# nka77/DAHiTra

Measured on AMD Instinct MI355X. Metric: image-pairs/s (256x256) train step, 1/2/4/8 MI355X + CPU ref, higher is better.
Workload: dtype bf16; 1 GPU; LEVIR-CD 256x256 synthetic pairs, base_transformer_pos_s4, bf16, batch 32 per GPU (global 32), fwd+focal+bwd+allreduce+AdamW; net_G=base_transformer_pos_s4, global_batch=32, img_size=256, parallelism=dp1, hip_graph=True, step_form=one graph (AdamW inside), attn_dtype=bf16

## Files before the change

dahitra_amd/csrc/norm.hip:

```cpp
#include "common.h"

namespace {

constexpr int BN_MAXG = 4;
__global__ void bn_finalize_kernel(const float* __restrict__ partial, int ntiles, int CP, int C, int G,
                                   double count, const float* __restrict__ gamma,
                                   const float* __restrict__ beta, float* __restrict__ running_mean,
                                   float* __restrict__ running_var, float momentum, float eps,
                                   float* __restrict__ mean_out, float* __restrict__ invstd_out,
                                   float* __restrict__ scale_out, float* __restrict__ shift_out,
                                   long long* __restrict__ nbt) {
    __shared__ double sm[BN_MAXG], sv[BN_MAXG], ps[4], pq[4];
    const int c = blockIdx.x;
    if (nbt && c == 0 && threadIdx.x == 0) *nbt += G;
    const int lane = threadIdx.x & 63, w = threadIdx.x >> 6, wpg = 4 / G;
    const int g = w / wpg, slice = w % wpg;
    const int tpg = ntiles / G;
    {
        double s = 0.0, q = 0.0, s2 = 0.0, q2 = 0.0;
        const float* p0 = partial + ((size_t)0 * CP + c) * ntiles + (size_t)g * tpg;
        const float* p1 = partial + ((size_t)1 * CP + c) * ntiles + (size_t)g * tpg;
        const int step = 64 * wpg;
        int t = slice * 64 + lane;
#pragma unroll 4
        for (; t + step < tpg; t += 2 * step) {
            s += (double)p0[t]; q += (double)p1[t];
            s2 += (double)p0[t + step]; q2 += (double)p1[t + step];
        }
        if (t < tpg) { s += (double)p0[t]; q += (double)p1[t]; }
        s += s2; q += q2;
#pragma unroll
        for (int o = 32; o > 0; o >>= 1) {
            s += __shfl_xor(s, o, 64);
            q += __shfl_xor(q, o, 64);
        }
        if (lane == 0) { ps[w] = s; pq[w] = q; }
        __syncthreads();
        if (lane == 0 && slice == 0) {
            s = 0.0; q = 0.0;
            for (int k = 0; k < wpg; ++k) { s += ps[g * wpg + k]; q += pq[g * wpg + k]; }
            const double mean = s / count;
            double var = q / count - mean * mean;
            if (var < 0.0) var = 0.0;
            const float invstd = (float)(1.0 / sqrt(var + (double)eps));
            const float sc = gamma[c] * invstd;
            mean_out[g * C + c] = (float)mean;
            invstd_out[g * C + c] = invstd;
            scale_out[g * C + c] = sc;
            shift_out[g * C + c] = beta[c] - (float)mean * sc;
            sm[g] = mean;
            sv[g] = count > 1.0 ? var * count / (count - 1.0) : var;
        }
    }
// ... 943 lines not shown
                              float momentum, float eps, float* mean, float* invstd, float* scale, float* shift,
                              long long* num_batches_tracked, void* stream) {
    DH_REQUIRE_BN_GROUPS("bn_finalize", groups);
    DH_REQUIRE(ntiles % groups == 0, "bn_finalize: ntiles=%d not divisible by groups=%d", ntiles, groups);
    hipLaunchKernelGGL(bn_finalize_kernel, dim3(C), dim3(256), 0, ST(stream), partial, ntiles, CP, C, groups, count,
                       gamma, beta, running_mean, running_var, momentum, eps, mean, invstd, scale, shift,
                       num_batches_tracked);
    DH_CHECK_LAUNCH("bn_finalize");
    return 0;
}

extern "C" int dh_bn_eval_params(const float* gamma, const float* beta, const float* running_mean,
                                 const float* running_var, float eps, int C, float* scale, float* shift,
                                 void* stream) {
    hipLaunchKernelGGL(bn_eval_params_kernel, dim3(dh_cdiv(C, 64)), dim3(64), 0, ST(stream), gamma, beta,
                       running_mean, running_var, eps, C, scale, shift);
    DH_CHECK_LAUNCH("bn_eval_params");
    return 0;
}

static int bn_apply_impl(int dtype, const void* x, const void* residual, void* y, const float* scale, const float* shift, long npix,
                         int C, int groups, int act, unsigned char* relu_bits, void* stream, const float* res_scale = nullptr,
                         const float* res_shift = nullptr) {
    const int V = dtype == DH_DTYPE_BF16 ? 8 : 4;
    DH_REQUIRE_BN_GROUPS("bn_apply", groups);
    DH_REQUIRE(C % V == 0 && npix % groups == 0, "bn_apply: C=%d npix=%ld groups=%d", C, npix, groups);
    DH_REQUIRE(!relu_bits || act == DH_ACT_RELU, "bn_apply: the ReLU mask bytes go with act = DH_ACT_RELU");
    DH_REQUIRE(!res_scale == !res_shift && (!res_scale || residual), "bn_apply: res_scale and res_shift go together, with a residual");
    const long nvec = npix * C / V, gvec = nvec / groups;
    (void)gvec;
    if (dtype == DH_DTYPE_BF16)
        launch_bn_apply<bf16>(x, residual, y, scale, shift, nvec, C, groups, act, ST(stream), relu_bits, res_scale, res_shift);
    else launch_bn_apply<float>(x, residual, y, scale, shift, nvec, C, groups, act, ST(stream), relu_bits, res_scale, res_shift);
    DH_CHECK_LAUNCH("bn_apply");
    return 0;
}
extern "C" int dh_bn_apply(int dtype, const void* x, const void* residual, void* y, const float* scale,
                           const float* shift, long npix, int C, int groups, int act, void* stream) {
    return bn_apply_impl(dtype, x, residual, y, scale, shift, npix, C, groups, act, nullptr, stream);
}
extern "C" int dh_bn_apply_bits(int dtype, const void* x, const void* residual, void* y, const float* scale, const float* shift,
                                long npix, int C, int groups, int act, unsigned char* relu_bits, void* stream) {
    DH_REQUIRE(relu_bits, "bn_apply_bits: relu_bits missing");
    return bn_apply_impl(dtype, x, residual, y, scale, shift, npix, C, groups, act, relu_bits, stream);
}

extern "C" int dh_bn_apply_res_affine(int dtype, const void* x, const void* residual, const float* res_scale, const float* res_shift,
                                      void* y, const float* scale, const float* shift, long npix, int C, int groups, int act,
                                      unsigned char* relu_bits, void* stream) {
    DH_REQUIRE(residual && res_scale && res_shift, "bn_apply_res_affine: residual, res_scale and res_shift are all required");
    return bn_apply_impl(dtype, x, residual, y, scale, shift, npix, C, groups, act, relu_bits, stream, res_scale, res_shift);
}

extern "C" long dh_stem_pool_bn_bwd_workspace_size(int C, int groups) { return (long)(768 / groups) * groups * 2 * C * 4; }
extern "C" int dh_stem_pool_bn_bwd_plus(const unsigned char* argmax, const void* dpool, const void* extra, const void* y,
                                        const float* mask_scale, const float* mask_shift, const float* mean, const float* invstd,
                                        const float* gamma, int N, int H, int W, int C, int groups, void* d, float* coef,
                                        float* dgamma, float* dbeta, int accumulate, void* workspace, void* stream);
extern "C" int dh_stem_pool_bn_bwd(const unsigned char* argmax, const void* dpool, const void* y, const float* mask_scale,
                                   const float* mask_shift, const float* mean, const float* invstd, const float* gamma, int N,
                                   int H, int W, int C, int groups, void* d, float* coef, float* dgamma, float* dbeta,
                                   int accumulate, void* workspace, void* stream) {
    return dh_stem_pool_bn_bwd_plus(argmax, dpool, nullptr, y, mask_scale, mask_shift, mean, invstd, gamma, N, H, W, C, groups, d,
                                    coef, dgamma, dbeta, accumulate, workspace, stream);
}
extern "C" int dh_stem_pool_bn_bwd_plus(const unsigned char* argmax, const void* dpool, const void* extra, const void* y,
                                        const float* mask_scale, const float* mask_shift, const float* mean, const float* invstd,
                                        const float* gamma, int N, int H, int W, int C, int groups, void* d, float* coef,
                                        float* dgamma, float* dbeta, int accumulate, void* workspace, void* stream) {
    DH_REQUIRE(C % 8 == 0 && 256 % (C / 8) == 0 && 2 * C <= 256, "stem_pool_bn_bwd: unsupported C=%d", C);
    DH_REQUIRE(groups >= 1 && groups <= BN_MAXG && N % groups == 0, "stem_pool_bn_bwd: N=%d groups=%d", N, groups);
    const int bpg = 768 / groups, OH = (H + 2 - 3) / 2 + 1, OW = (W + 2 - 3) / 2 + 1;
    float* partial = reinterpret_cast<float*>(workspace);
    hipLaunchKernelGGL(pool_bn_bwd_reduce_kernel, dim3(groups * bpg), dim3(256), 0, ST(stream), argmax, (const bf16*)dpool,
                       (const bf16*)extra, (const bf16*)y, mask_scale, mask_shift, (bf16*)d, partial, N / groups, H, W, C, OH, OW, bpg);
    hipLaunchKernelGGL(bn_bwd_finalize_coef_kernel, dim3(C), dim3(64 * groups), 0, ST(stream), partial, bpg, groups, C, mean, invstd,
                       gamma, 1.0f / (float)((long)(N / groups) * H * W), coef, dgamma, dbeta, accumulate);
    DH_CHECK_LAUNCH("stem_pool_bn_bwd");
    return 0;
}

extern "C" long dh_bn_bwd_workspace_size(long npix, int C, int groups) {
    const int bpg = 1024 / groups;
    return ((long)groups * bpg * 2 * C + (long)groups * 2 * C) * 4;
}

static int bn_bwd_impl(int dtype, const void* dout, const void* out_relu, bool bits, const void* x, const float* mean,
                       const float* invstd, const float* gamma, long npix, int C, int groups, void* dx,
                       void* dres, float* dgamma, float* dbeta, int accumulate, const float* mask_scale,
                       const float* mask_shift, void* workspace, void* stream) {
    DH_REQUIRE_BN_GROUPS("bn_bwd", groups);
    DH_REQUIRE(!(out_relu && mask_scale), "bn_bwd: give the ReLU mask either as out_relu or as mask_scale/shift");
    DH_REQUIRE(!bits || out_relu, "bn_bwd: mask bytes missing");
    const int V = dtype == DH_DTYPE_BF16 ? 8 : 4;
    DH_REQUIRE(C % V == 0 && (256 * V) % C == 0, "bn_bwd: unsupported C=%d", C);
    DH_REQUIRE(npix % groups == 0, "bn_bwd: npix=%ld not divisible by groups=%d", npix, groups);
    const int bpg = 1024 / groups;
    const long ppg = npix / groups;
    float* partial = reinterpret_cast<float*>(workspace);
    float* sums = partial + (long)groups * bpg * 2 * C;
    const long nvec = npix * C / V;
    if (dtype == DH_DTYPE_BF16) {
        launch_bn_bwd_reduce<bf16>(dout, out_relu, x, mean, invstd, C, ppg, bpg, groups, partial, mask_scale, mask_shift, ST(stream), bits);
        hipLaunchKernelGGL(bn_bwd_finalize_kernel, dim3(C), dim3(64 * groups), 0, ST(stream), partial, bpg, groups, C, sums,
                           dgamma, dbeta, accumulate);
        launch_bn_bwd_apply<bf16>(dout, out_relu, x, mean, invstd, gamma, sums, ppg, nvec, C, groups, dx, dres, mask_scale,
                                  mask_shift, ST(stream), bits);
    } else {
        launch_bn_bwd_reduce<float>(dout, out_relu, x, mean, invstd, C, ppg, bpg, groups, partial, mask_scale, mask_shift, ST(stream), bits);
        hipLaunchKernelGGL(bn_bwd_finalize_kernel, dim3(C), dim3(64 * groups), 0, ST(stream), partial, bpg, groups, C, sums,
                           dgamma, dbeta, accumulate);
        launch_bn_bwd_apply<float>(dout, out_relu, x, mean, invstd, gamma, sums, ppg, nvec, C, groups, dx, dres, mask_scale,
                                   mask_shift, ST(stream), bits);
    }
    DH_CHECK_LAUNCH("bn_bwd");
    return 0;
}
extern "C" int dh_bn_bwd(int dtype, const void* dout, const void* out_relu, const void* x, const float* mean,
                         const float* invstd, const float* gamma, long npix, int C, int groups, void* dx,
                         void* dres, float* dgamma, float* dbeta, int accumulate, const float* mask_scale,
                         const float* mask_shift, void* workspace, void* stream) {
    return bn_bwd_impl(dtype, dout, out_relu, false, x, mean, invstd, gamma, npix, C, groups, dx, dres, dgamma, dbeta, accumulate,
                       mask_scale, mask_shift, workspace, stream);
}
extern "C" int dh_bn_bwd_bits(int dtype, const void* dout, const unsigned char* relu_bits, const void* x, const float* mean,
                              const float* invstd, const float* gamma, long npix, int C, int groups, void* dx,
                              void* dres, float* dgamma, float* dbeta, int accumulate, void* workspace, void* stream) {
    DH_REQUIRE(relu_bits, "bn_bwd_bits: relu_bits missing");
// ... 171 lines not shown
```

dahitra_amd/csrc/pointwise.hip:

```cpp
#include "common.h"

namespace {

inline int ew_grid(long n, int block) {
    long g = (n + block - 1) / block;
    return (int)(g > 8192 ? 8192 : (g < 1 ? 1 : g));
}
#define GSL(i, n) for (long i = (long)blockIdx.x * blockDim.x + threadIdx.x; i < (n); i += (long)gridDim.x * blockDim.x)

template <typename T>
__global__ void nchw_to_nhwc_kernel(const float* __restrict__ src, T* __restrict__ dst, int N, int C, long HW, int CP) {
    const long total = (long)N * HW * CP;
    GSL(i, total) {
        const int c = (int)(i % CP);
        const long p = (i / CP) % HW;
        const long n = i / (CP * HW);
        stf(dst + i, c < C ? src[(n * C + c) * HW + p] : 0.f);
    }
}
template <typename T>
__global__ void nchw_to_nhwc_piece_kernel(const float* __restrict__ src, T* __restrict__ dst, int N, int C, long HW) {
    constexpr int V = V16<T>::N;
    const long total = (long)N * HW;
    GSL(i, total) {
        const long p = i % HW, n = i / HW;
        float v[V];
#pragma unroll
        for (int c = 0; c < V; ++c) v[c] = c < C ? src[(n * C + c) * HW + p] : 0.f;
        stv(dst + i * V, v);
    }
}
template <typename T>
__global__ void nhwc_to_nchw_kernel(const T* __restrict__ src, float* __restrict__ dst, int N, int C, long HW) {
    const long total = (long)N * HW * C;
    GSL(i, total) {
        const long p = i % HW;
        const int c = (int)((i / HW) % C);
        const long n = i / (HW * C);
        dst[i] = ldf(src + (n * HW + p) * C + c);
    }
}

template <typename T, int CP>
__global__ __launch_bounds__(256) void head_dgrad3x3_kernel(const T* __restrict__ dy, const float* __restrict__ w_oihw,
                                                            T* __restrict__ dx, int N, int H, int W, int NC) {
    __shared__ __attribute__((aligned(16))) float sw[9 * 8 * 32];
    for (int i = threadIdx.x; i < 9 * NC * 32; i += blockDim.x) {
        const int ci = i & 31, co = (i >> 5) % NC, tap = i / (32 * NC);
        sw[i] = w_oihw[((size_t)co * 32 + ci) * 9 + tap];
    }
    __syncthreads();
    const long total = (long)N * H * W;
    for (long px = (long)blockIdx.x * blockDim.x + threadIdx.x; px < total; px += (long)gridDim.x * blockDim.x) {
// ... 1097 lines not shown
    DH_REQUIRE(C % V == 0, "cat_halves: C=%d must be a multiple of %d", C, V);
    const long n = P * (2 * C / V);
    if (dtype == DH_DTYPE_BF16) {
        if (inverse) hipLaunchKernelGGL((cat_halves_kernel<bf16, true>), dim3(ew_grid(n, 256)), dim3(256), 0, ST(stream), (bf16*)t, (bf16*)cat, C, P);
        else hipLaunchKernelGGL((cat_halves_kernel<bf16, false>), dim3(ew_grid(n, 256)), dim3(256), 0, ST(stream), (bf16*)t, (bf16*)cat, C, P);
    } else {
        if (inverse) hipLaunchKernelGGL((cat_halves_kernel<float, true>), dim3(ew_grid(n, 256)), dim3(256), 0, ST(stream), (float*)t, (float*)cat, C, P);
        else hipLaunchKernelGGL((cat_halves_kernel<float, false>), dim3(ew_grid(n, 256)), dim3(256), 0, ST(stream), (float*)t, (float*)cat, C, P);
    }
    DH_CHECK_LAUNCH("cat_halves");
    return 0;
}
extern "C" int dh_add(int dtype, const void* a, const void* b, void* y, long n, void* stream) {
    DH_REQUIRE(n % 4 == 0, "add: n must be a multiple of 4");
    const long nv = n / 4;
    if (dtype == DH_DTYPE_BF16 && n % 8 == 0) hipLaunchKernelGGL(add16_kernel<bf16>, dim3(ew_grid(n / 8, 256)), dim3(256), 0, ST(stream), (const bf16*)a, (const bf16*)b, (bf16*)y, n / 8);
    else if (dtype == DH_DTYPE_BF16) hipLaunchKernelGGL(add_kernel<bf16>, dim3(ew_grid(nv, 256)), dim3(256), 0, ST(stream), (const bf16*)a, (const bf16*)b, (bf16*)y, nv);
    else hipLaunchKernelGGL(add_kernel<float>, dim3(ew_grid(nv, 256)), dim3(256), 0, ST(stream), (const float*)a, (const float*)b, (float*)y, nv);
    DH_CHECK_LAUNCH("add");
    return 0;
}
extern "C" int dh_add_pos(int dtype, const void* x, const float* pos, void* y, int N, long HW, int C, void* stream) {
    const long n = (long)N * HW * C;
    if (dtype == DH_DTYPE_BF16 && C % 8 == 0) hipLaunchKernelGGL(add_pos16_kernel<bf16>, dim3(ew_grid(n / 8, 256)), dim3(256), 0, ST(stream), (const bf16*)x, pos, (bf16*)y, N, HW, C);
    else if (dtype == DH_DTYPE_BF16) hipLaunchKernelGGL(add_pos_kernel<bf16>, dim3(ew_grid(n, 256)), dim3(256), 0, ST(stream), (const bf16*)x, pos, (bf16*)y, N, HW, C);
    else hipLaunchKernelGGL(add_pos_kernel<float>, dim3(ew_grid(n, 256)), dim3(256), 0, ST(stream), (const float*)x, pos, (float*)y, N, HW, C);
    DH_CHECK_LAUNCH("add_pos");
    return 0;
}
extern "C" int dh_add_pos_bwd(int dtype, const void* dy, float* dpos, int N, long HW, int C, int accumulate, void* stream) {
    const long n = HW * C;
    if (dtype == DH_DTYPE_BF16 && C == 32) hipLaunchKernelGGL(add_pos_bwd32_kernel, dim3((unsigned)((HW + 15) / 16)), dim3(256), 0, ST(stream), (const bf16*)dy, dpos, N, HW, accumulate);
    else if (dtype == DH_DTYPE_BF16) hipLaunchKernelGGL(add_pos_bwd_kernel<bf16>, dim3(ew_grid(n, 256)), dim3(256), 0, ST(stream), (const bf16*)dy, dpos, N, HW, C, accumulate);
    else hipLaunchKernelGGL(add_pos_bwd_kernel<float>, dim3(ew_grid(n, 256)), dim3(256), 0, ST(stream), (const float*)dy, dpos, N, HW, C, accumulate);
    DH_CHECK_LAUNCH("add_pos_bwd");
    return 0;
}
extern "C" int dh_act_bwd(int dtype, const void* dy, const void* ref, void* dx, long n, int act, void* stream) {
    DH_REQUIRE(n % 4 == 0 && (act == DH_ACT_RELU || act == DH_ACT_GELU), "act_bwd: bad arguments");
    const long nv = n / 4;
    if (dtype == DH_DTYPE_BF16 && n % 8 == 0) hipLaunchKernelGGL(act_bwd16_kernel<bf16>, dim3(ew_grid(n / 8, 256)), dim3(256), 0, ST(stream), (const bf16*)dy, (const bf16*)ref, (bf16*)dx, n / 8, act);
    else if (dtype == DH_DTYPE_BF16) hipLaunchKernelGGL(act_bwd_kernel<bf16>, dim3(ew_grid(nv, 256)), dim3(256), 0, ST(stream), (const bf16*)dy, (const bf16*)ref, (bf16*)dx, nv, act);
    else hipLaunchKernelGGL(act_bwd_kernel<float>, dim3(ew_grid(nv, 256)), dim3(256), 0, ST(stream), (const float*)dy, (const float*)ref, (float*)dx, nv, act);
    DH_CHECK_LAUNCH("act_bwd");
    return 0;
}
extern "C" int dh_maxpool3x3s2_fwd(int dtype, const void* x, void* y, unsigned char* argmax, int N, int H, int W, int C,
                                   const float* bn_scale, const float* bn_shift, int groups, void* stream) {
    DH_REQUIRE(!bn_scale || (bn_shift && groups > 0 && N % groups == 0), "maxpool: bn_scale needs bn_shift and groups | N");
    const int V = dtype == DH_DTYPE_BF16 ? 8 : 4;
    DH_REQUIRE(C % V == 0, "maxpool: C=%d must be a multiple of %d", C, V);
    const int OH = (H + 2 - 3) / 2 + 1, OW = (W + 2 - 3) / 2 + 1;
    const long n = (long)N * OH * OW * (C / V);
    if (dtype == DH_DTYPE_BF16) hipLaunchKernelGGL(maxpool_fwd_kernel<bf16>, dim3(ew_grid(n, 256)), dim3(256), 0, ST(stream), (const bf16*)x, (bf16*)y, argmax, N, H, W, C, OH, OW, bn_scale, bn_shift, groups);
    else hipLaunchKernelGGL(maxpool_fwd_kernel<float>, dim3(ew_grid(n, 256)), dim3(256), 0, ST(stream), (const float*)x, (float*)y, argmax, N, H, W, C, OH, OW, bn_scale, bn_shift, groups);
    DH_CHECK_LAUNCH("maxpool_fwd");
    return 0;
}
extern "C" int dh_maxpool3x3s2_bwd(int dtype, const unsigned char* argmax, const void* dy, void* dx, int N, int H, int W, int C, void* stream) {
    const int V = dtype == DH_DTYPE_BF16 ? 8 : 4;
    DH_REQUIRE(C % V == 0, "maxpool: C=%d must be a multiple of %d", C, V);
    const int OH = (H + 2 - 3) / 2 + 1, OW = (W + 2 - 3) / 2 + 1;
    const long n = (long)N * ((H + 1) / 2) * ((W + 1) / 2) * (C / V);
    if (dtype == DH_DTYPE_BF16) hipLaunchKernelGGL(maxpool_bwd_kernel<bf16>, dim3(ew_grid(n, 256)), dim3(256), 0, ST(stream), argmax, (const bf16*)dy, (bf16*)dx, N, H, W, C, OH, OW);
    else hipLaunchKernelGGL(maxpool_bwd_kernel<float>, dim3(ew_grid(n, 256)), dim3(256), 0, ST(stream), argmax, (const float*)dy, (float*)dx, N, H, W, C, OH, OW);
    DH_CHECK_LAUNCH("maxpool_bwd");
    return 0;
}
extern "C" int dh_upsample2_nearest_fwd(int dtype, const void* x, void* y, int N, int H, int W, int C, void* stream) {
    const int V = dtype == DH_DTYPE_BF16 ? 8 : 4;
    DH_REQUIRE(C % V == 0, "upsample2: C=%d must be a multiple of %d", C, V);
    const long n = (long)N * 4 * H * W * (C / V);
    if (dtype == DH_DTYPE_BF16) hipLaunchKernelGGL(up2_fwd_kernel<bf16>, dim3(ew_grid(n, 256)), dim3(256), 0, ST(stream), (const bf16*)x, (bf16*)y, N, H, W, C);
    else hipLaunchKernelGGL(up2_fwd_kernel<float>, dim3(ew_grid(n, 256)), dim3(256), 0, ST(stream), (const float*)x, (float*)y, N, H, W, C);
    DH_CHECK_LAUNCH("up2_fwd");
    return 0;
}
extern "C" int dh_upsample2_nearest_bwd(int dtype, const void* dy, void* dx, int N, int H, int W, int C, void* stream) {
    const int V = dtype == DH_DTYPE_BF16 ? 8 : 4;
    DH_REQUIRE(C % V == 0, "upsample2: C=%d must be a multiple of %d", C, V);
    const long n = (long)N * H * W * (C / V);
    if (dtype == DH_DTYPE_BF16) hipLaunchKernelGGL(up2_bwd_kernel<bf16>, dim3(ew_grid(n, 256)), dim3(256), 0, ST(stream), (const bf16*)dy, (bf16*)dx, N, H, W, C);
    else hipLaunchKernelGGL(up2_bwd_kernel<float>, dim3(ew_grid(n, 256)), dim3(256), 0, ST(stream), (const float*)dy, (float*)dx, N, H, W, C);
    DH_CHECK_LAUNCH("up2_bwd");
    return 0;
}
extern "C" int dh_absdiff_upsample4_fwd(int dtype, const void* a, const void* b, void* y, int N, int H, int W, int C, void* stream) {
    const int V = dtype == DH_DTYPE_BF16 ? 8 : 4;
    DH_REQUIRE(C % V == 0, "absdiff_upsample4: C=%d must be a multiple of %d", C, V);
    const long n = (long)N * H * W * (C / V);
    if (dtype == DH_DTYPE_BF16) hipLaunchKernelGGL(absdiff_up4_fwd_kernel<bf16>, dim3(ew_grid(n, 256)), dim3(256), 0, ST(stream), (const bf16*)a, (const bf16*)b, (bf16*)y, N, H, W, C);
    else hipLaunchKernelGGL(absdiff_up4_fwd_kernel<float>, dim3(ew_grid(n, 256)), dim3(256), 0, ST(stream), (const float*)a, (const float*)b, (float*)y, N, H, W, C);
    DH_CHECK_LAUNCH("absdiff_up4_fwd");
    return 0;
}
extern "C" int dh_absdiff_upsample4_bwd(int dtype, const void* a, const void* b, const void* dy, void* da, void* db, int N, int H, int W, int C, void* stream) {
    const int V = dtype == DH_DTYPE_BF16 ? 8 : 4;
    DH_REQUIRE(C % V == 0, "absdiff_upsample4: C=%d must be a multiple of %d", C, V);
    const long n = (long)N * H * W * (C / V);
    if (dtype == DH_DTYPE_BF16) hipLaunchKernelGGL(absdiff_up4_bwd_kernel<bf16>, dim3(ew_grid(n, 256)), dim3(256), 0, ST(stream), (const bf16*)a, (const bf16*)b, (const bf16*)dy, (bf16*)da, (bf16*)db, N, H, W, C);
    else hipLaunchKernelGGL(absdiff_up4_bwd_kernel<float>, dim3(ew_grid(n, 256)), dim3(256), 0, ST(stream), (const float*)a, (const float*)b, (const float*)dy, (float*)da, (float*)db, N, H, W, C);
    DH_CHECK_LAUNCH("absdiff_up4_bwd");
    return 0;
}
extern "C" int dh_absdiff_up4_combine(const float* partial, const void* a, const void* b, void* da, void* db, int N, int H, int W,
                                      void* stream) {
    DH_REQUIRE(H % 2 == 0 && W % 4 == 0, "absdiff_up4_combine: coarse map %dx%d must tile into 8x16 fine tiles", H, W);
    const long n = (long)N * H * W * 4;
    hipLaunchKernelGGL(absdiff_up4_combine_kernel, dim3(ew_grid(n, 256)), dim3(256), 0, ST(stream), partial, (const bf16*)a,
                       (const bf16*)b, (bf16*)da, (bf16*)db, N, H, W);
    DH_CHECK_LAUNCH("absdiff_up4_combine");
    return 0;
}
extern "C" int dh_absdiff(int dtype, const void* a, const void* b, void* y, long n, void* stream) {
    if (dtype == DH_DTYPE_BF16) hipLaunchKernelGGL(absdiff_kernel<bf16>, dim3(ew_grid(n, 256)), dim3(256), 0, ST(stream), (const bf16*)a, (const bf16*)b, (bf16*)y, n);
    else hipLaunchKernelGGL(absdiff_kernel<float>, dim3(ew_grid(n, 256)), dim3(256), 0, ST(stream), (const float*)a, (const float*)b, (float*)y, n);
    DH_CHECK_LAUNCH("absdiff");
// ... 176 lines not shown
```

dahitra_amd/ops.py:

```python
import bisect
import ctypes
import math
import os
import sys

import numpy as np
import torch

from . import _lib

ACT_NONE, ACT_RELU, ACT_GELU = 0, 1, 2
_DT = {torch.float32: 0, torch.bfloat16: 1}
_vp = ctypes.c_void_p


def dt(t):
    try:
        return _DT[t.dtype]
    except KeyError:
        raise TypeError("dahitra_amd: unsupported activation dtype %s" % t.dtype)


def set_f32_mma_mode(mode):
    _lib.check(_lib.lib().dh_set_f32_mma_mode(int(mode)), "dh_set_f32_mma_mode")
# ... 1043 lines not shown
    assert cat.is_contiguous()
    if cat.dtype == torch.bfloat16 and (c2 // 2) % 8 == 0 and _ew_record(EW_SPLIT_HALVES, cat, None, t, c2 // 2, 0, n * h * w):
        return t
    _call("dh_cat_halves", dt(cat), P(t), P(cat), c2 // 2, n * h * w, 1, S())
    return t


def add(a, b):
    y = torch.empty_like(a)
    _call("dh_add", dt(a), P(a), P(b), P(y), a.numel(), S())
    return y


def add_pos(x, pos):
    N, H, W, C = x.shape
    y = torch.empty_like(x)
    assert x.is_contiguous() and pos.is_contiguous()
    if x.dtype == torch.bfloat16 and C % 8 == 0 and _ew_record(EW_ADD_POS, x, pos, y, N, C, H * W):
        return y
    _call("dh_add_pos", dt(x), P(x), P(pos), P(y), N, H * W, C, S())
    return y


def add_pos_bwd(dy, dpos, accumulate=False):
    N, H, W, C = dy.shape
    assert dy.is_contiguous() and dpos.is_contiguous()
    if dy.dtype == torch.bfloat16 and C == 32 and _ew_record(EW_ADD_POS_BWD, dy, None, dpos, N, int(accumulate), H * W):
        return
    _call("dh_add_pos_bwd", dt(dy), P(dy), P(dpos), N, H * W, C, accumulate, S())


def act_bwd(dy, ref, act):
    dx = torch.empty_like(dy)
    _call("dh_act_bwd", dt(dy), P(dy), P(ref), P(dx), dy.numel(), act, S())
    return dx


def maxpool(x, want_arg=False, bn=None):
    N, H, W, C = x.shape
    y = torch.empty(N, (H - 1) // 2 + 1, (W - 1) // 2 + 1, C, dtype=x.dtype, device=x.device)
    arg = torch.empty(y.shape, dtype=torch.uint8, device=x.device) if want_arg else None
    sc, sh, groups = bn if bn is not None else (None, None, 0)
    _call("dh_maxpool3x3s2_fwd", dt(x), P(x), P(y), P(arg), N, H, W, C, P(sc), P(sh), groups, S())
    return (y, arg) if want_arg else y


def maxpool_bwd(arg, dy, in_shape):
    N, H, W, C = in_shape
    dx = torch.empty(N, H, W, C, dtype=dy.dtype, device=dy.device)
    _call("dh_maxpool3x3s2_bwd", dt(dy), P(arg), P(dy), P(dx), N, H, W, C, S())
    return dx


def upsample2(x):
    N, H, W, C = x.shape
    y = torch.empty(N, 2 * H, 2 * W, C, dtype=x.dtype, device=x.device)
    _call("dh_upsample2_nearest_fwd", dt(x), P(x), P(y), N, H, W, C, S())
    return y


def upsample2_bwd(dy):
    N, H2, W2, C = dy.shape
    dx = torch.empty(N, H2 // 2, W2 // 2, C, dtype=dy.dtype, device=dy.device)
    _call("dh_upsample2_nearest_bwd", dt(dy), P(dy), P(dx), N, H2 // 2, W2 // 2, C, S())
    return dx


def absdiff_upsample4(a, b):
    N, H, W, C = a.shape
    y = torch.empty(N, 4 * H, 4 * W, C, dtype=a.dtype, device=a.device)
    _call("dh_absdiff_upsample4_fwd", dt(a), P(a), P(b), P(y), N, H, W, C, S())
    return y


def absdiff_upsample4_bwd(a, b, dy):
    N, H, W, C = a.shape
    da, db = torch.empty_like(a), torch.empty_like(b)
    _call("dh_absdiff_upsample4_bwd", dt(a), P(a), P(b), P(dy), P(da), P(db), N, H, W, C, S())
    return da, db


def conv3x3_dgrad_through_up4(dy, wdgrad, a, b, da=None, db=None):
    N, H, W, C = a.shape
    assert C == 32 and a.dtype == torch.bfloat16 and dy.shape[:3] == (N, 4 * H, 4 * W) and wdgrad.shape[-2] == 32
    L = _lib.lib()
    partial = torch.empty(L.dh_conv3x3_dgrad_up4_partial_floats(N, 4 * H, 4 * W), dtype=torch.float32, device=a.device)
    with _Prof("conv_mfma<bf16,ks3,s1,nt32>", 2.0 * N * 16 * H * W * 32 * dy.shape[-1] * 9, _nb(dy, wdgrad, partial)):
        _call("dh_conv3x3_dgrad_up4", dt(dy), P(dy), P(wdgrad), N, 4 * H, 4 * W, dy.shape[-1], P(partial), S())
    da = torch.empty_like(a) if da is None else da
    db = torch.empty_like(b) if db is None else db
    _call("dh_absdiff_up4_combine", P(partial), P(a), P(b), P(da), P(db), N, H, W, S())
    return da, db


def absdiff(a, b):
    y = torch.empty_like(a)
    _call("dh_absdiff", dt(a), P(a), P(b), P(y), a.numel(), S())
    return y


def absdiff_bwd(a, b, dy, da, db, accumulate=True):
    _call("dh_absdiff_bwd", dt(a), P(a), P(b), P(dy), P(da), P(db), a.numel(), accumulate, S())


def colsum(x2d, out, accumulate=False):
    C = x2d.shape[-1]
# ... 1263 lines not shown
```

include/dahitra_hip.h:

```cpp
#ifndef DAHITRA_HIP_H
#define DAHITRA_HIP_H
#ifdef __cplusplus
extern "C" {
#endif

#define DH_F32 0
#define DH_BF16 1
#define DH_ACT_NONE 0
#define DH_ACT_RELU 1
#define DH_ACT_GELU 2

int dh_abi_version(void);
const char* dh_last_error(void);
void dh_set_error(const char* msg);

int dh_conv2d_fwd(int dtype, const void* x, const void* w_packed, void* y, const float* bias,
                  const void* residual, float* stats_partial, int N, int H, int W, int Cin, int OH, int OW,
                  int Cout, int CoutPad, int ks, int stride, int pad, int act, int npix_valid,
                  long w_image_stride, void* y_preact, int dilation, const void* gate_out, const void* gate_y,
                  const float* gate_mean, const float* gate_invstd, int gate_groups, const float* in_scale,
                  const float* in_shift, int in_groups, int phase_mode, const void* w_frag, void* stream);
int dh_conv2d_fwd_num_tiles(int dtype, int N, int OH, int OW, int Cin, int ks, int stride);
int dh_conv2d_fwd_describe(int entry, int dtype, int N, int H, int W, int Cin, int OH, int OW, int Cout, int CoutPad, int ks, int stride,
                           int pad, int act, int npix_valid, long w_image_stride, int dilation, int gate_groups, int in_groups,
// ... 125 lines not shown
                             const int* params, const int* blur, int N, int H, int W, int h, int w, float* out_a,
                             float* out_b, unsigned char* out_l, void* stream);
int dh_xbd_augment_u8(const unsigned char* pre, const unsigned char* post, const unsigned char* pre_mask,
                      const unsigned char* post_label, const int* idx, const int* params, const int* coef, int N, int H, int W,
                      int S, int mode, float* out_img, unsigned char* out_msk, unsigned char* out_lbl, void* stream);
int dh_xbd_augment_jitter_tiles(int S);
int dh_xbd_augment_jitter_u8(const unsigned char* pre, const unsigned char* post, const unsigned char* pre_mask,
                             const unsigned char* post_label, const int* idx, const int* params, const int* coef,
                             const int* jitter_host, int N, int H, int W, int S, int mode, float* out_img, unsigned char* out_msk,
                             unsigned char* out_lbl, void* workspace, long workspace_bytes, void* stream);
int dh_xbd_augment_warp_tile_h(void);
int dh_xbd_augment_warp_tile_w(void);
int dh_xbd_augment_warp_u8(const unsigned char* pre, const unsigned char* post, const unsigned char* post_label, const int* idx,
                           const int* params, const int* tab, int N, int H, int W, int S, float* out_img, unsigned char* out_msk,
                           void* stream);
int dh_xbd_unet_colour_tile(void);
int dh_xbd_unet_colour_ws_bytes(int J, int S, long* bytes);
int dh_xbd_unet_colour_u8(float* img, const int* jobs, const unsigned char* noise, int N, int S, int J, int K, void* workspace,
                          long workspace_bytes, void* stream);
int dh_nchw_to_nhwc(int dtype, const float* src, void* dst, int N, int C, long HW, int CP, void* stream);
int dh_head_dgrad3x3(int dtype, const void* dy, int CP, const float* w_oihw, int NC, void* dx, int N, int H, int W,
                     void* stream);
int dh_head_dgrad3x3_relu(const void* dy, const float* w_oihw, int NC, const void* relu_out, void* dx, int N, int H, int W,
                          void* stream);
int dh_head_dgrad3x3_bn_blocks(int N, int H, int W, int groups);
int dh_head_dgrad3x3_bn(const void* dy, const float* w_oihw, int NC, const void* y, const float* mask_scale, const float* mask_shift,
                        const float* mean, const float* invstd, int groups, void* g, float* partial, int N, int H, int W,
                        void* stream);
int dh_head_bn_bwd_blocks(int N, int H, int W, int groups);
long dh_head_bn_bwd_workspace_size(int N, int H, int W, int groups);
int dh_head_dlogits_pack(int dtype, const float* dlogits_nchw, int N, int NC, int H, int W, void* dlp, void* stream);
int dh_head_bn_bwd(int dtype, const void* dlp, const float* w_oihw, int NC, const void* y, const float* mask_scale, const float* mask_shift,
                   const float* mean, const float* invstd, const float* gamma, int groups, void* dx, float* dgamma, float* dbeta,
                   float* dw, float* db, int accumulate, int N, int H, int W, void* workspace, void* stream);
int dh_head_relu_bwd(int dtype, const void* dlp, const float* w_oihw, int NC, const void* relu_out, void* dx, float* dw, float* db,
                     int accumulate, int N, int H, int W, void* workspace, void* stream);
int dh_head_fwd_supported(int NC, int W);
int dh_head_fwd(int dtype, const void* x, const float* w_oihw, const float* bias, int NC, const float* in_scale, const float* in_shift,
                int in_groups, float* logits_nchw, int N, int H, int W, void* stream);
enum { DH_EW_ADD_POS = 1, DH_EW_CAT_HALVES = 2, DH_EW_SPLIT_HALVES = 3, DH_EW_ABSDIFF_HALVES = 4, DH_EW_ABSDIFF_HALVES_BWD = 5,
       DH_EW_ADD_POS_BWD = 6 };
int dh_ew_multi(int n, const int* op, const void* const* a, const void* const* b, void* const* c, const int* i0, const int* i1,
                const long* l0, void* stream);
int dh_nhwc_to_nchw(int dtype, const void* src, float* dst, int N, int C, long HW, void* stream);
int dh_copy_channels(int dtype, const void* src, int Cs, int sc0, void* dst, int Cd, int dc0, int Cn, long P, void* stream);
int dh_cat_halves(int dtype, void* t, void* cat, int C, long P, int inverse, void* stream);
int dh_add(int dtype, const void* a, const void* b, void* y, long n, void* stream);
int dh_add_pos(int dtype, const void* x, const float* pos, void* y, int N, long HW, int C, void* stream);
int dh_add_pos_bwd(int dtype, const void* dy, float* dpos, int N, long HW, int C, int accumulate, void* stream);
int dh_act_bwd(int dtype, const void* dy, const void* ref, void* dx, long n, int act, void* stream);
int dh_maxpool3x3s2_fwd(int dtype, const void* x, void* y, unsigned char* argmax, int N, int H, int W, int C,
                        const float* bn_scale, const float* bn_shift, int groups, void* stream);
int dh_maxpool3x3s2_bwd(int dtype, const unsigned char* argmax, const void* dy, void* dx, int N, int H, int W, int C, void* stream);
int dh_upsample2_nearest_fwd(int dtype, const void* x, void* y, int N, int H, int W, int C, void* stream);
int dh_upsample2_nearest_bwd(int dtype, const void* dy, void* dx, int N, int H, int W, int C, void* stream);
int dh_absdiff_upsample4_fwd(int dtype, const void* a, const void* b, void* y, int N, int H, int W, int C, void* stream);
int dh_absdiff_upsample4_bwd(int dtype, const void* a, const void* b, const void* dy, void* da, void* db, int N, int H, int W, int C, void* stream);
int dh_absdiff(int dtype, const void* a, const void* b, void* y, long n, void* stream);
int dh_absdiff_bwd(int dtype, const void* a, const void* b, const void* dy, void* da, void* db, long n, int accumulate, void* stream);
int dh_colsum(int dtype, const void* x, long P, int C, float* out, int accumulate, void* workspace, void* stream);
int dh_cast_from_f32(int dtype, const float* src, void* dst, long n, void* stream);
int dh_cast_to_f32(int dtype, const void* src, float* dst, long n, int accumulate, void* stream);

int dh_tokenizer_fwd(int dtype, const void* x, const float* wa, const float* pos, int S, int B, int HW, int L,
                     float* logits, float* stats, float* pooled, float* tok_cat, void* workspace, void* stream);
long dh_tokenizer_fwd_workspace_size(int S, int HW, int L);
int dh_tokenizer_bwd(int dtype, const void* x, const float* wa, int S, int B, int HW, int L, const float* logits,
                     const float* stats, const float* pooled, const float* dtok_cat, void* dx_accum, float* dwa,
                     float* dpos, int accumulate, void* workspace, void* stream);
long dh_tokenizer_bwd_workspace_size(int S, int HW, int L);
int dh_xattn_prep_fwd(int dtype, const void* tok, long tok_bstride, long tok_sstride, int B, int S, int L, int heads,
                      int dim_head, int HLP, float scale, float eps, const float* ln_g, const float* ln_b,
                      const float* wq, const void* wkT, const void* wvT, const void* woT, float* mn, float* mstats,
                      float* k, float* v, void* kq, void* kqT, void* vo, void* voT, void* stream);
int dh_xattn_prep_fwd_stack(int dtype, const void* tok, long tok_bstride, long tok_sstride, int B, int S, int L, int heads,
                            int dim_head, int HLP, float scale, float eps, int layers, long param_stride,
                            const float* ln_g, const float* ln_b, const float* wq, const void* wkT, const void* wvT,
                            const void* woT, float* mn, float* mstats, float* k, float* v, void* kq, void* kqT, void* vo,
                            void* voT, void* stream);
int dh_xattn_prep_mfma_supported(int dtype, int S, int L, int heads, int dim_head, int HLP);
int dh_xattn_prep_fwd_stack_mfma(const void* tok, long tok_bstride, long tok_sstride, int B, int S, int heads, int dim_head,
                                 int HLP, float scale, float eps, int layers, long param_stride, const float* ln_g,
                                 const float* ln_b, const float* wk, const float* wv, const float* wo, const void* wqT,
                                 float* mn, float* mstats, float* k, float* v, void* kq, void* kqT, void* vo, void* voT,
                                 void* stream);
int dh_xattn_prep_bwd_stack_mfma(const void* tok, void* dtok_accum, long tok_bstride, long tok_sstride, int B, int S, int heads,
                                 int dim_head, int HLP, float scale, int layers, long param_stride, const float* ln_g,
                                 const float* wq, const void* woT, const void* wkT, const void* wvT, const float* mn,
                                 const float* mstats, const float* k, const float* v, const float* dkq, const float* dvoT,
                                 float* dk, float* dv, float* dln_g, float* dln_b, float* dwq, float* dwk, float* dwv,
                                 float* dwo, int accumulate, void* workspace, void* stream);
int dh_xattn_prep_bwd_stack(int dtype, const void* tok, void* dtok_accum, long tok_bstride, long tok_sstride, int B, int S,
                            int L, int heads, int dim_head, int HLP, float scale, int layers, long param_stride,
                            const float* ln_g, const void* wqT, const float* wk, const float* wv, const float* wo,
                            const float* mn, const float* mstats, const float* k, const float* v, const float* dkq,
                            const float* dvoT, float* dk, float* dv, float* dln_g, float* dln_b, float* dwq, float* dwk,
                            float* dwv, float* dwo, int accumulate, void* workspace, void* stream);
long dh_xattn_prep_bwd_stack_workspace_size(int S, int L, int layers);
int dh_xattn_prep_bwd(int dtype, const void* tok, void* dtok_accum, long tok_bstride, long tok_sstride, int B, int S,
                      int L, int heads, int dim_head, int HLP, float scale, const float* ln_g, const void* wqT,
                      const float* wk, const float* wv, const float* wo, const float* mn, const float* mstats,
                      const float* k, const float* v, const float* dkq, const float* dvoT, float* dk, float* dv,
                      float* dln_g, float* dln_b, float* dwq, float* dwk, float* dwv, float* dwo, int accumulate,
                      void* workspace, void* stream);
long dh_xattn_prep_bwd_workspace_size(int S);
int dh_softmax_groups_fwd(int dtype, const void* x, void* y, long rows, int heads, int L, int HLP, void* stream);
// ... 183 lines not shown
```

Measured before the change: 9570 image-pairs/s.

## Add row-tiled maxpool 3x3s2 forward/backward kernels with fused BN and reuse

Adds new tiled kernels for the stem 3x3 stride-2 maxpool. Each thread walks a column strip of 8 output rows and carries overlapping input rows and the top row's packed max-keys in registers, so shared rows are not reloaded. The forward pass fuses BN+ReLU and computes argmax by packing position codes into the low bits of the bf16 key. The backward and BN-backward paths gather gradients per input 2x2 block instead of scattering, and the BN-backward kernel writes per-block partial sums for the finalize kernel. A runtime toggle falls back to the old kernels; the risk is more code complexity and tie-breaking that differs in subtle ways from the original argmax.

Result: no change. 9656 image-pairs/s (median of 6 runs) (+0.9%).

```diff
diff --git a/dahitra_amd/csrc/norm.hip b/dahitra_amd/csrc/norm.hip
--- a/dahitra_amd/csrc/norm.hip
+++ b/dahitra_amd/csrc/norm.hip
@@ -1,4 +1,5 @@
 #include "common.h"
+#include "pool_tiled.h"
 
 namespace {
 
@@ -1048,7 +1049,10 @@
     return bn_apply_impl(dtype, x, residual, y, scale, shift, npix, C, groups, act, relu_bits, stream, res_scale, res_shift);
 }
 
-extern "C" long dh_stem_pool_bn_bwd_workspace_size(int C, int groups) { return (long)(768 / groups) * groups * 2 * C * 4; }
+extern "C" long dh_stem_pool_bn_bwd_workspace_size(int C, int groups) {
+    const long generic = (long)(768 / groups) * groups, tiled = (long)(POOL_TILED_WGS / groups) * groups;
+    return (generic > tiled ? generic : tiled) * 2 * C * 4;
+}
 extern "C" int dh_stem_pool_bn_bwd_plus(const unsigned char* argmax, const void* dpool, const void* extra, const void* y,
                                         const float* mask_scale, const float* mask_shift, const float* mean, const float* invstd,
                                         const float* gamma, int N, int H, int W, int C, int groups, void* d, float* coef,
@@ -1066,10 +1070,14 @@
                                         float* dgamma, float* dbeta, int accumulate, void* workspace, void* stream) {
     DH_REQUIRE(C % 8 == 0 && 256 % (C / 8) == 0 && 2 * C <= 256, "stem_pool_bn_bwd: unsupported C=%d", C);
     DH_REQUIRE(groups >= 1 && groups <= BN_MAXG && N % groups == 0, "stem_pool_bn_bwd: N=%d groups=%d", N, groups);
-    const int bpg = 768 / groups, OH = (H + 2 - 3) / 2 + 1, OW = (W + 2 - 3) / 2 + 1;
+    int bpg = 768 / groups;
+    const int OH = (H + 2 - 3) / 2 + 1, OW = (W + 2 - 3) / 2 + 1;
     float* partial = reinterpret_cast<float*>(workspace);
-    hipLaunchKernelGGL(pool_bn_bwd_reduce_kernel, dim3(groups * bpg), dim3(256), 0, ST(stream), argmax, (const bf16*)dpool,
-                       (const bf16*)extra, (const bf16*)y, mask_scale, mask_shift, (bf16*)d, partial, N / groups, H, W, C, OH, OW, bpg);
+    if (pool_tiled_bn_bwd(argmax, dpool, extra, y, mask_scale, mask_shift, d, partial, N, H, W, C, groups, ST(stream)))
+        bpg = POOL_TILED_WGS / groups;
+    else
+        hipLaunchKernelGGL(pool_bn_bwd_reduce_kernel, dim3(groups * bpg), dim3(256), 0, ST(stream), argmax, (const bf16*)dpool,
+                           (const bf16*)extra, (const bf16*)y, mask_scale, mask_shift, (bf16*)d, partial, N / groups, H, W, C, OH, OW, bpg);
     hipLaunchKernelGGL(bn_bwd_finalize_coef_kernel, dim3(C), dim3(64 * groups), 0, ST(stream), partial, bpg, groups, C, mean, invstd,
                        gamma, 1.0f / (float)((long)(N / groups) * H * W), coef, dgamma, dbeta, accumulate);
     DH_CHECK_LAUNCH("stem_pool_bn_bwd");
diff --git a/dahitra_amd/csrc/pointwise.hip b/dahitra_amd/csrc/pointwise.hip
--- a/dahitra_amd/csrc/pointwise.hip
+++ b/dahitra_amd/csrc/pointwise.hip
@@ -1,4 +1,5 @@
 #include "common.h"
+#include "pool_tiled.h"
 
 namespace {
 
@@ -1202,7 +1203,8 @@
     DH_REQUIRE(C % V == 0, "maxpool: C=%d must be a multiple of %d", C, V);
     const int OH = (H + 2 - 3) / 2 + 1, OW = (W + 2 - 3) / 2 + 1;
     const long n = (long)N * OH * OW * (C / V);
-    if (dtype == DH_DTYPE_BF16) hipLaunchKernelGGL(maxpool_fwd_kernel<bf16>, dim3(ew_grid(n, 256)), dim3(256), 0, ST(stream), (const bf16*)x, (bf16*)y, argmax, N, H, W, C, OH, OW, bn_scale, bn_shift, groups);
+    if (dtype == DH_DTYPE_BF16 && pool_tiled_fwd(x, y, argmax, N, H, W, C, bn_scale, bn_shift, groups, ST(stream))) {}
+    else if (dtype == DH_DTYPE_BF16) hipLaunchKernelGGL(maxpool_fwd_kernel<bf16>, dim3(ew_grid(n, 256)), dim3(256), 0, ST(stream), (const bf16*)x, (bf16*)y, argmax, N, H, W, C, OH, OW, bn_scale, bn_shift, groups);
     else hipLaunchKernelGGL(maxpool_fwd_kernel<float>, dim3(ew_grid(n, 256)), dim3(256), 0, ST(stream), (const float*)x, (float*)y, argmax, N, H, W, C, OH, OW, bn_scale, bn_shift, groups);
     DH_CHECK_LAUNCH("maxpool_fwd");
     return 0;
@@ -1212,7 +1214,8 @@
     DH_REQUIRE(C % V == 0, "maxpool: C=%d must be a multiple of %d", C, V);
     const int OH = (H + 2 - 3) / 2 + 1, OW = (W + 2 - 3) / 2 + 1;
     const long n = (long)N * ((H + 1) / 2) * ((W + 1) / 2) * (C / V);
-    if (dtype == DH_DTYPE_BF16) hipLaunchKernelGGL(maxpool_bwd_kernel<bf16>, dim3(ew_grid(n, 256)), dim3(256), 0, ST(stream), argmax, (const bf16*)dy, (bf16*)dx, N, H, W, C, OH, OW);
+    if (dtype == DH_DTYPE_BF16 && pool_tiled_bwd(argmax, dy, dx, N, H, W, C, ST(stream))) {}
+    else if (dtype == DH_DTYPE_BF16) hipLaunchKernelGGL(maxpool_bwd_kernel<bf16>, dim3(ew_grid(n, 256)), dim3(256), 0, ST(stream), argmax, (const bf16*)dy, (bf16*)dx, N, H, W, C, OH, OW);
     else hipLaunchKernelGGL(maxpool_bwd_kernel<float>, dim3(ew_grid(n, 256)), dim3(256), 0, ST(stream), argmax, (const float*)dy, (float*)dx, N, H, W, C, OH, OW);
     DH_CHECK_LAUNCH("maxpool_bwd");
     return 0;
diff --git a/dahitra_amd/csrc/pool_tiled.h b/dahitra_amd/csrc/pool_tiled.h
--- /dev/null
+++ b/dahitra_amd/csrc/pool_tiled.h
@@ -0,0 +1,10 @@
+#pragma once
+#include <hip/hip_runtime.h>
+
+constexpr int POOL_TILED_WGS = 1024;
+
+bool pool_tiled_fwd(const void* x, void* y, unsigned char* argmax, int N, int H, int W, int C, const float* bn_scale,
+                    const float* bn_shift, int groups, hipStream_t st);
+bool pool_tiled_bwd(const unsigned char* argmax, const void* dy, void* dx, int N, int H, int W, int C, hipStream_t st);
+bool pool_tiled_bn_bwd(const unsigned char* argmax, const void* dpool, const void* extra, const void* y, const float* mask_scale,
+                       const float* mask_shift, void* d, float* partial, int N, int H, int W, int C, int groups, hipStream_t st);
diff --git a/dahitra_amd/csrc/pool_tiled.hip b/dahitra_amd/csrc/pool_tiled.hip
--- /dev/null
+++ b/dahitra_amd/csrc/pool_tiled.hip
@@ -0,0 +1,284 @@
+#include "common.h"
+#include "pool_tiled.h"
+#include "dahitra_hip.h"
+
+namespace {
+
+constexpr int PT_R = 8;
+
+int g_pool_tiled = 1;
+
+struct PtTile { long n; int r0, col; };
+__device__ __forceinline__ PtTile pt_tile(int t, int g, int npg, int TR, int TC, int T, int tx) {
+    PtTile p;
+    p.n = (long)g * npg + t / (TR * TC);
+    p.r0 = (t / TC) % TR * PT_R;
+    p.col = (t % TC) * T + tx;
+    return p;
+}
+
+__device__ __forceinline__ void pt_row_keys(const uint4 (&raw)[3], const float (&sc)[8], const float (&sh)[8], unsigned ml,
+                                            unsigned cl, unsigned mr, unsigned (&hk)[8]) {
+#pragma unroll
+    for (int q = 0; q < 3; ++q) {
+        const unsigned m = q == 0 ? ml : (q == 1 ? 0xffff0u : mr), code = q == 0 ? cl : (q == 1 ? 1u : 0u);
+        float v[8];
+        unpack16(raw[q], v);
+#pragma unroll
+        for (int e = 0; e < 4; ++e) {
+            const unsigned pk = f2bf2(fmaxf(v[2 * e] * sc[2 * e] + sh[2 * e], 0.f), fmaxf(v[2 * e + 1] * sc[2 * e + 1] + sh[2 * e + 1], 0.f));
+            const unsigned klo = ((pk << 4) & m) | code, khi = ((pk >> 12) & m) | code;
+            hk[2 * e] = q == 0 ? klo : (klo > hk[2 * e] ? klo : hk[2 * e]);
+            hk[2 * e + 1] = q == 0 ? khi : (khi > hk[2 * e + 1] ? khi : hk[2 * e + 1]);
+        }
+    }
+}
+
+__global__ __launch_bounds__(256) void maxpool_bn_tiled_fwd_kernel(const bf16* __restrict__ x, bf16* __restrict__ y,
+                                                                   unsigned char* __restrict__ arg, int npg, int H, int W, int C,
+                                                                   int OH, int OW, const float* __restrict__ bn_scale,
+                                                                   const float* __restrict__ bn_shift) {
+    const int vn = C / 8, T = 256 / vn, g = blockIdx.y;
+    const int c = ((int)threadIdx.x % vn) * 8, tx = (int)threadIdx.x / vn;
+    float sc[8], sh[8];
+#pragma unroll
+    for (int j = 0; j < 8; ++j) { sc[j] = bn_scale[g * C + c + j]; sh[j] = bn_shift[g * C + c + j]; }
+    const int TR = (OH + PT_R - 1) / PT_R, TC = (OW + T - 1) / T, tiles = npg * TR * TC;
+    for (int t = blockIdx.x; t < tiles; t += gridDim.x) {
+        const PtTile tl = pt_tile(t, g, npg, TR, TC, T, tx);
+        const bool act = tl.col < OW;
+        const int ox = act ? tl.col : OW - 1, oy0 = tl.r0;
+        const bool vl = ox > 0, vr = 2 * ox + 1 < W;
+        const unsigned ml = vl ? 0xffff0u : 0u, cl = vl ? 2u : 0u, mr = vr ? 0xffff0u : 0u;
+        const bf16* xn = x + tl.n * H * W * C + c;
+        const long o0 = (long)(2 * ox - (vl ? 1 : 0)) * C, o1 = (long)(2 * ox) * C, o2 = (long)(2 * ox + (vr ? 1 : 0)) * C;
+        auto ldrow = [&](int iy, uint4 (&raw)[3]) {
+            const bf16* p = xn + (long)iy * W * C;
+            raw[0] = *reinterpret_cast<const uint4*>(p + o0);
+            raw[1] = *reinterpret_cast<const uint4*>(p + o1);
+            raw[2] = *reinterpret_cast<const uint4*>(p + o2);
+        };
+        unsigned top[8];
+#pragma unroll
+        for (int j = 0; j < 8; ++j) top[j] = 0u;
+        uint4 ra[3], rb[3];
+        if (oy0 > 0) {
+            ldrow(2 * oy0 - 1, ra);
+            pt_row_keys(ra, sc, sh, ml, cl, mr, top);
+#pragma unroll
+            for (int j = 0; j < 8; ++j) top[j] |= 8u;
+        }
+        ldrow(2 * oy0, ra);
+        ldrow(min(2 * oy0 + 1, H - 1), rb);
+#pragma unroll
+        for (int r = 0; r < PT_R; ++r) {
+            const int oy = oy0 + r;
+            if (oy >= OH) break;
+            uint4 na[3], nb[3];
+            if (r + 1 < PT_R) {
+                ldrow(min(2 * oy + 2, H - 1), na);
+                ldrow(min(2 * oy + 3, H - 1), nb);
+            }
+            unsigned ka[8], kb[8], k[8];
+            pt_row_keys(ra, sc, sh, ml, cl, mr, ka);
+            pt_row_keys(rb, sc, sh, ml, cl, mr, kb);
+            const bool vb = 2 * oy + 1 < H;
+#pragma unroll
+            for (int j = 0; j < 8; ++j) {
+                if (!vb) kb[j] = 0u;
+                ka[j] |= 4u;
+                k[j] = top[j] > ka[j] ? top[j] : ka[j];
+                k[j] = kb[j] > k[j] ? kb[j] : k[j];
+                top[j] = kb[j] | 8u;
+            }
+            if (act) {
+                const long o = ((tl.n * OH + oy) * OW + ox) * C + c;
+                uint4 v;
+                v.x = (k[0] >> 4) | ((k[1] << 12) & 0xffff0000u);
+                v.y = (k[2] >> 4) | ((k[3] << 12) & 0xffff0000u);
+                v.z = (k[4] >> 4) | ((k[5] << 12) & 0xffff0000u);
+                v.w = (k[6] >> 4) | ((k[7] << 12) & 0xffff0000u);
+                *reinterpret_cast<uint4*>(y + o) = v;
+                if (arg) {
+                    unsigned long long bits = 0;
+#pragma unroll
+                    for (int j = 0; j < 8; ++j) {
+                        const unsigned f = k[j] & 15u;
+                        bits |= (unsigned long long)(8u - f + (f >> 2)) << (8 * j);
+                    }
+                    *reinterpret_cast<unsigned long long*>(arg + o) = bits;
+                }
+            }
+            if (r + 1 < PT_R) {
+#pragma unroll
+                for (int q = 0; q < 3; ++q) { ra[q] = na[q]; rb[q] = nb[q]; }
+            }
+        }
+    }
+}
+
+template <int V> struct PtPiece;
+template <> struct PtPiece<8> { typedef uint4 P; typedef unsigned long long B; };
+template <> struct PtPiece<4> { typedef uint2 P; typedef unsigned B; };
+__device__ __forceinline__ void pt_unpack(const uint4& u, float (&o)[8]) { unpack16(u, o); }
+__device__ __forceinline__ void pt_unpack(const uint2& u, float (&o)[4]) {
+    o[0] = __uint_as_float(u.x << 16); o[1] = __uint_as_float(u.x & 0xffff0000u);
+    o[2] = __uint_as_float(u.y << 16); o[3] = __uint_as_float(u.y & 0xffff0000u);
+}
+__device__ __forceinline__ void pt_store(bf16* p, const float (&o)[8]) { stv(p, o); }
+__device__ __forceinline__ void pt_store(bf16* p, const float (&o)[4]) { st4(p, o); }
+template <int V> struct PtWin { typename PtPiece<V>::B bits; typename PtPiece<V>::P d; };
+template <int V>
+__device__ __forceinline__ void pt_ld_win(const unsigned char* __restrict__ arg, const bf16* __restrict__ dy, long o, bool in, PtWin<V>& w) {
+    typedef typename PtPiece<V>::B B;
+    typedef typename PtPiece<V>::P P;
+    const B b = *reinterpret_cast<const B*>(arg + o);
+    const P v = *reinterpret_cast<const P*>(dy + o);
+    w.bits = in ? b : ~B(0);
+    w.d = in ? v : P{};
+}
+
+template <bool BN, bool EX, int V>
+__global__ __launch_bounds__(256, 4) void pool_tiled_bwd_kernel(const unsigned char* __restrict__ arg, const bf16* __restrict__ dpool,
+                                                                         const bf16* __restrict__ extra, const bf16* __restrict__ y,
+                                                                         const float* __restrict__ mscale, const float* __restrict__ mshift,
+                                                                         bf16* __restrict__ d, float* __restrict__ partial, int npg, int H,
+                                                                         int W, int C, int OH, int OW) {
+    typedef typename PtPiece<V>::P P;
+    static_assert(BN || !EX, "extra belongs to the stem tail");
+    __shared__ float red[BN ? 2 : 1][BN ? 256 : 1][V];
+    const int vn = C / V, T = 256 / vn, g = blockIdx.y, BH = (H + 1) / 2, BW = (W + 1) / 2;
+    const int c = ((int)threadIdx.x % vn) * V, tx = (int)threadIdx.x / vn;
+    float ms[V], mh[V], s1[V], s2[V];
+#pragma unroll
+    for (int j = 0; j < V; ++j) {
+        ms[j] = BN ? mscale[g * C + c + j] : 0.f; mh[j] = BN ? mshift[g * C + c + j] : 0.f;
+        s1[j] = s2[j] = 0.f;
+    }
+    const int TR = (BH + PT_R - 1) / PT_R, TC = (BW + T - 1) / T, tiles = npg * TR * TC;
+    for (int t = blockIdx.x; t < tiles; t += gridDim.x) {
+        const PtTile tl = pt_tile(t, g, npg, TR, TC, T, tx);
+        const bool act = tl.col < BW;
+        const int bx = act ? tl.col : BW - 1, by0 = tl.r0;
+        const bool vx1 = bx + 1 < OW;
+        const bool px1 = 2 * bx + 1 < W;
+        const long wn = tl.n * OH * OW * C + (long)bx * C + c, pn = tl.n * H * W * C + (long)2 * bx * C + c;
+        const int wx1 = vx1 ? C : 0, pc1 = px1 ? C : 0;
+        PtWin<V> w[2][2];
+        pt_ld_win(arg, dpool, wn + (long)by0 * OW * C, true, w[0][0]);
+        pt_ld_win(arg, dpool, wn + (long)by0 * OW * C + wx1, vx1, w[0][1]);
+#pragma unroll 1
+        for (int r = 0; r < PT_R; ++r) {
+            const int by = by0 + r;
+            if (by >= BH) break;
+            const bool vy1 = by + 1 < OH, py1 = 2 * by + 1 < H;
+            const long wrow = wn + (long)(by + (vy1 ? 1 : 0)) * OW * C;
+            pt_ld_win(arg, dpool, wrow, vy1, w[1][0]);
+            pt_ld_win(arg, dpool, wrow + wx1, vy1 && vx1, w[1][1]);
+            const long prow[2] = {pn + (long)(2 * by) * W * C, pn + (long)(2 * by + (py1 ? 1 : 0)) * W * C};
+            P yr[2][2], er[2][2];
+#pragma unroll
+            for (int a = 0; a < 2; ++a)
+#pragma unroll
+                for (int bb = 0; bb < 2; ++bb) {
+                    if (BN) yr[a][bb] = *reinterpret_cast<const P*>(y + prow[a] + bb * pc1);
+                    if (EX) er[a][bb] = *reinterpret_cast<const P*>(extra + prow[a] + bb * pc1);
+                }
+#pragma unroll
+            for (int a = 0; a < 2; ++a)
+#pragma unroll
+                for (int bb = 0; bb < 2; ++bb) {
+                    const bool pv = act && (a == 0 || py1) && (bb == 0 || px1);
+                    float gs[V];
+#pragma unroll
+                    for (int j = 0; j < V; ++j) gs[j] = 0.f;
+#pragma unroll
+                    for (int wy = 0; wy <= a; ++wy)
+#pragma unroll
+                        for (int wx = 0; wx <= bb; ++wx) {
+                            const unsigned kk = (a + 1 - 2 * wy) * 3 + (bb + 1 - 2 * wx);
+                            float dv[V];
+                            pt_unpack(w[wy][wx].d, dv);
+#pragma unroll
+                            for (int j = 0; j < V; ++j)
+                                if (((w[wy][wx].bits >> (8 * j)) & 0xff) == kk) gs[j] += dv[j];
+                        }
+                    if (BN) {
+                        float yv[V];
+                        pt_unpack(yr[a][bb], yv);
+                        if (EX) {
+                            float ev[V];
+                            pt_unpack(er[a][bb], ev);
+#pragma unroll
+                            for (int j = 0; j < V; ++j) gs[j] += ev[j];
+                        }
+#pragma unroll
+                        for (int j = 0; j < V; ++j) {
+                            const float gm = (yv[j] * ms[j] + mh[j]) > 0.f ? gs[j] : 0.f;
+                            gs[j] = gm;
+                            const float gp = pv ? gm : 0.f;
+                            s1[j] += gp;
+                            s2[j] += gp * yv[j];
+                        }
+                    }
+                    if (pv) pt_store(d + prow[a] + bb * pc1, gs);
+                }
+            w[0][0] = w[1][0];
+            w[0][1] = w[1][1];
+        }
+    }
+    if (BN) {
+#pragma unroll
+        for (int j = 0; j < V; ++j) { red[0][threadIdx.x][j] = s1[j]; red[1][threadIdx.x][j] = s2[j]; }
+        __syncthreads();
+        if ((int)threadIdx.x < 2 * C) {
+            const int which = threadIdx.x / C, ch = threadIdx.x % C, piece = ch / V, j = ch % V;
+            float s = 0.f;
+            for (int k = piece; k < 256; k += vn) s += red[which][k][j];
+            const size_t slots = (size_t)gridDim.x * gridDim.y;
+            partial[((size_t)which * C + ch) * slots + (size_t)blockIdx.y * gridDim.x + blockIdx.x] = s;
+        }
+    }
+}
+
+constexpr int PT_BNV = 4;
+
+bool pt_serves(int C, int V = 8) { return g_pool_tiled != 0 && C >= 8 && C % 8 == 0 && 256 % (C / V) == 0; }
+
+}
+
+bool pool_tiled_fwd(const void* x, void* y, unsigned char* argmax, int N, int H, int W, int C, const float* bn_scale,
+                    const float* bn_shift, int groups, hipStream_t st) {
+    if (!pt_serves(C) || !bn_scale || groups > POOL_TILED_WGS) return false;
+    const int OH = (H - 1) / 2 + 1, OW = (W - 1) / 2 + 1;
+    hipLaunchKernelGGL(maxpool_bn_tiled_fwd_kernel, dim3(POOL_TILED_WGS / groups, groups), dim3(256), 0, st, (const bf16*)x,
+                       (bf16*)y, argmax, N / groups, H, W, C, OH, OW, bn_scale, bn_shift);
+    return true;
+}
+bool pool_tiled_bwd(const unsigned char* argmax, const void* dy, void* dx, int N, int H, int W, int C, hipStream_t st) {
+    if (!pt_serves(C)) return false;
+    const int OH = (H - 1) / 2 + 1, OW = (W - 1) / 2 + 1;
+    hipLaunchKernelGGL((pool_tiled_bwd_kernel<false, false, 8>), dim3(POOL_TILED_WGS, 1), dim3(256), 0, st, argmax, (const bf16*)dy,
+                       (const bf16*)nullptr, (const bf16*)nullptr, (const float*)nullptr, (const float*)nullptr, (bf16*)dx,
+                       (float*)nullptr, N, H, W, C, OH, OW);
+    return true;
+}
+bool pool_tiled_bn_bwd(const unsigned char* argmax, const void* dpool, const void* extra, const void* y, const float* mask_scale,
+                       const float* mask_shift, void* d, float* partial, int N, int H, int W, int C, int groups, hipStream_t st) {
+    if (!pt_serves(C, PT_BNV) || 2 * C > 256) return false;
+    const int OH = (H - 1) / 2 + 1, OW = (W - 1) / 2 + 1;
+    const dim3 grid(POOL_TILED_WGS / groups, groups);
+    if (extra)
+        hipLaunchKernelGGL((pool_tiled_bwd_kernel<true, true, PT_BNV>), grid, dim3(256), 0, st, argmax, (const bf16*)dpool, (const bf16*)extra,
+                           (const bf16*)y, mask_scale, mask_shift, (bf16*)d, partial, N / groups, H, W, C, OH, OW);
+    else
+        hipLaunchKernelGGL((pool_tiled_bwd_kernel<true, false, PT_BNV>), grid, dim3(256), 0, st, argmax, (const bf16*)dpool, (const bf16*)nullptr,
+                           (const bf16*)y, mask_scale, mask_shift, (bf16*)d, partial, N / groups, H, W, C, OH, OW);
+    return true;
+}
+
+extern "C" int dh_pool_tiled_mode(int mode) {
+    const int prev = g_pool_tiled;
+    g_pool_tiled = mode != 0 ? 1 : 0;
+    return prev;
+}
diff --git a/dahitra_amd/ops.py b/dahitra_amd/ops.py
--- a/dahitra_amd/ops.py
+++ b/dahitra_amd/ops.py
@@ -1119,6 +1119,10 @@
     return dx
 
 
+def pool_tiled_mode(mode):
+    return int(_lib.lib().dh_pool_tiled_mode(int(mode)))
+
+
 def upsample2(x):
     N, H, W, C = x.shape
     y = torch.empty(N, 2 * H, 2 * W, C, dtype=x.dtype, device=x.device)
diff --git a/include/dahitra_hip.h b/include/dahitra_hip.h
--- a/include/dahitra_hip.h
+++ b/include/dahitra_hip.h
@@ -201,6 +201,7 @@
 int dh_maxpool3x3s2_fwd(int dtype, const void* x, void* y, unsigned char* argmax, int N, int H, int W, int C,
                         const float* bn_scale, const float* bn_shift, int groups, void* stream);
 int dh_maxpool3x3s2_bwd(int dtype, const unsigned char* argmax, const void* dy, void* dx, int N, int H, int W, int C, void* stream);
+int dh_pool_tiled_mode(int mode);
 int dh_upsample2_nearest_fwd(int dtype, const void* x, void* y, int N, int H, int W, int C, void* stream);
 int dh_upsample2_nearest_bwd(int dtype, const void* dy, void* dx, int N, int H, int W, int C, void* stream);
 int dh_absdiff_upsample4_fwd(int dtype, const void* a, const void* b, void* y, int N, int H, int W, int C, void* stream);
```
